# XuyangBai/D3Feat

Hardware: NVIDIA H100
Metric: points/sec through KPFCNN encoder (higher is better)
Workload: dtype f32

## Files before the change

d3feat_b200/csrc/kpconv.cu:

```cuda
#include <stdlib.h>

#include "ops.cuh"

namespace d3f {


constexpr int kS1Warps = 4;
constexpr int kWStride = 20;
constexpr int kKMax = 16;

struct Stage1Params {
  const float* q;
  const float4* s4;
  const int* idx;
  const float* feat;
  int count_nn;
  const float* Kp;
  const float* offsets;
  const float* modulations;
  int Nq, Ns, H, Cin;
  int n0, n1;
  const int* order;
  float extent;
  float inv_scale;
// ... 271 lines not shown
#pragma unroll
        for (int k = 0; k < K; ++k) w[k] = (k == kmin) ? w[k] : 0.f;
      }
      const bool keep = real && qvalid && (!DEFORM || in_range);
#pragma unroll
      for (int kq = 0; kq < KP / 4; ++kq)
        *reinterpret_cast<float4*>(&wq[sl * kWStride + 4 * kq]) =
            keep ? make_float4(w[4 * kq], w[4 * kq + 1], w[4 * kq + 2], w[4 * kq + 3]) : make_float4(0.f, 0.f, 0.f, 0.f);
      if (c0 == 0 && p.count_nn) nn_count += __popc((__ballot_sync(0xffffffffu, sp.w > 0.f) >> gshift) & gmask);
      unsigned m = (__ballot_sync(0xffffffffu, keep) >> gshift) & gmask;
      int cnt = __popc(m);
      if (QPW >= 2) cnt = max(cnt, __shfl_xor_sync(0xffffffffu, cnt, 16));
      if (QPW >= 4) cnt = max(cnt, __shfl_xor_sync(0xffffffffu, cnt, 8));
      __syncwarp();

      constexpr int kUnroll = CPL == 4 ? 2 : 4;
      for (int it = 0; it < cnt; it += kUnroll) {
        int hh[kUnroll];
        float f[kUnroll][CPL];
#pragma unroll
        for (int u = 0; u < kUnroll; ++u) {
          const bool act = m != 0;
          hh[u] = act ? __ffs(m) - 1 : 0;
          m &= m - 1;
          const int idh = __shfl_sync(0xffffffffu, id, (int)gshift + hh[u]);
          const float* fp = p.feat + (size_t)idh * p.Cin + c;
          if (CPL == 4) {
            float4 t = act ? __ldg(reinterpret_cast<const float4*>(fp)) : make_float4(0.f, 0.f, 0.f, 0.f);
            f[u][0] = t.x; f[u][1] = t.y; f[u][2 % CPL] = t.z; f[u][3 % CPL] = t.w;
          } else {
            float2 t = act ? __ldg(reinterpret_cast<const float2*>(fp)) : make_float2(0.f, 0.f);
            f[u][0] = t.x; f[u][1] = t.y;
          }
        }
#pragma unroll
        for (int u = 0; u < kUnroll; ++u) {
          const float4* wp = reinterpret_cast<const float4*>(&wq[hh[u] * kWStride]);
          float2 wpair[KP / 2];
#pragma unroll
          for (int kq = 0; kq < KP / 4; ++kq) {
            float4 t = wp[kq];
            wpair[2 * kq] = make_float2(t.x, t.y);
            wpair[2 * kq + 1] = make_float2(t.z, t.w);
          }
#pragma unroll
          for (int v = 0; v < CPL; ++v) {
            const float2 fd = make_float2(f[u][v], f[u][v]);
#pragma unroll
            for (int j = 0; j < KP / 2; ++j) acc[j][v] = ffma2(wpair[j], fd, acc[j][v]);
          }
        }
      }
      __syncwarp();
    }

    if (qvalid) {
      float* dst = p.wf + (size_t)(n - p.n0) * K * p.Cin + c;
#pragma unroll
      for (int k = 0; k < K; ++k) {
        const float mod = (DEFORM && p.modulations) ? p.modulations[(size_t)nq * K + k] : 1.f;
        float o[CPL];
#pragma unroll
        for (int v = 0; v < CPL; ++v) o[v] = ((k & 1) ? acc[k / 2][v].y : acc[k / 2][v].x) * mod;
        if (CPL == 4) *reinterpret_cast<float4*>(dst + (size_t)k * p.Cin) = make_float4(o[0], o[1], o[2 % CPL], o[3 % CPL]);
        else *reinterpret_cast<float2*>(dst + (size_t)k * p.Cin) = make_float2(o[0], o[1]);
      }
    }
  }
  if (p.inv_nn != nullptr && qvalid && sl == 0) p.inv_nn[n - p.n0] = 1.f / (float)max(nn_count, 1);
}

__device__ __forceinline__ void mma_tf32(float (&c)[4], const unsigned (&a)[4], unsigned b0, unsigned b1) {
  asm volatile("mma.sync.aligned.m16n8k8.row.col.f32.tf32.tf32.f32 {%0,%1,%2,%3}, {%4,%5,%6,%7}, {%8,%9}, {%0,%1,%2,%3};"
               : "+f"(c[0]), "+f"(c[1]), "+f"(c[2]), "+f"(c[3])
               : "r"(a[0]), "r"(a[1]), "r"(a[2]), "r"(a[3]), "r"(b0), "r"(b1));
}
__device__ __forceinline__ void split3(float x, unsigned& hi, unsigned& lo) {
  hi = (__float_as_uint(x) + 0x1000u) & 0xFFFFE000u;
  lo = __float_as_uint(x - __uint_as_float(hi));
}


template <int NT>
__global__ void __launch_bounds__(kS1Warps * 32, NT == 4 ? 8 : (NT == 8 ? 5 : 3))
kpconv_stage1_fast_kernel(Stage1Params p) {
  const int Ns_ = dyn_rows(p.Ns, p.ns_dev), n1_ = min(p.n1, dyn_rows(p.Nq, p.nq_dev));
  constexpr int K = 15;
  static_assert(NT % 4 == 0, "one float4 per four n-tiles");
  const int lane = threadIdx.x & 31, warp = threadIdx.x >> 5;
  const int g = lane >> 2, t = lane & 3;
  const int n = p.n0 + blockIdx.x * kS1Warps + warp;
  if (n >= n1_) return;
  const int kA = g, kB = g + 8;
  const bool validB = kB < K;
  const float kax = p.Kp[3 * kA], kay = p.Kp[3 * kA + 1], kaz = p.Kp[3 * kA + 2];
  const float kbx = validB ? p.Kp[3 * kB] : 1e6f, kby = validB ? p.Kp[3 * kB + 1] : 1e6f,
              kbz = validB ? p.Kp[3 * kB + 2] : 1e6f;
  const int qid = p.order ? p.order[n] : n;
  const float qx = p.q[3 * (size_t)qid], qy = p.q[3 * (size_t)qid + 1], qz = p.q[3 * (size_t)qid + 2];
  const int* row = p.idx + (size_t)qid * p.H + t;
  const float inv_scale = p.inv_scale;
  const unsigned Ns = (unsigned)Ns_;
  const unsigned Cin = (unsigned)p.Cin;
  int cnt = 0;

  constexpr int CCH = NT * 8;
  for (int c0 = blockIdx.y * CCH; c0 < p.Cin; c0 += gridDim.y * CCH) {
    float acc[NT][4];
#pragma unroll
    for (int i = 0; i < NT; ++i) acc[i][0] = acc[i][1] = acc[i][2] = acc[i][3] = 0.f;
    const float* fcol = p.feat + c0 + NT * g;
    asm volatile("" : "+l"(fcol));

    unsigned ida_n = Ns, idb_n = Ns;
    if (t < p.H) ida_n = (unsigned)__ldg(row);
    if (t + 4 < p.H) idb_n = (unsigned)__ldg(row + 4);
    for (int h0 = 0; h0 < p.H; h0 += 8) {
      const unsigned ida = min(ida_n, Ns);
      const unsigned idb = min(idb_n, Ns);
      ida_n = Ns;
      idb_n = Ns;
      if (h0 + 8 + t < p.H) ida_n = (unsigned)__ldg(row + h0 + 8);
      if (h0 + 12 + t < p.H) idb_n = (unsigned)__ldg(row + h0 + 12);
      const float4 spa = __ldg(&p.s4[ida]), spb = __ldg(&p.s4[idb]);
      float fa[NT], fb[NT];
#pragma unroll
      for (int v = 0; v < NT; v += 4) {
        float4 x = make_float4(0.f, 0.f, 0.f, 0.f), y = make_float4(0.f, 0.f, 0.f, 0.f);
        if (ida < Ns) x = __ldg(reinterpret_cast<const float4*>(fcol + (size_t)(ida * Cin) + v));
        if (idb < Ns) y = __ldg(reinterpret_cast<const float4*>(fcol + (size_t)(idb * Cin) + v));
        fa[v] = x.x; fa[v + 1] = x.y; fa[v + 2] = x.z; fa[v + 3] = x.w;
        fb[v] = y.x; fb[v + 1] = y.y; fb[v + 2] = y.z; fb[v + 3] = y.w;
      }
      if (c0 == 0) cnt += (spa.w > 0.f ? 1 : 0) + (spb.w > 0.f ? 1 : 0);
      const float rax = spa.x - qx, ray = spa.y - qy, raz = spa.z - qz;
      const float rbx = spb.x - qx, rby = spb.y - qy, rbz = spb.z - qz;
      auto weight = [&](float rx, float ry, float rz, float kx, float ky, float kz) {
        const float dx = rx - kx, dy = ry - ky, dz = rz - kz;
        const float d2 = fmaf(dz, dz, fmaf(dy, dy, fmaf(dx, dx, 1e-10f)));
        return fmaxf(fmaf(-sqrt_approx(d2), inv_scale, 1.f), 0.f);
      };
      unsigned ah[4], al[4];
      split3(weight(rax, ray, raz, kax, kay, kaz), ah[0], al[0]);
      split3(weight(rax, ray, raz, kbx, kby, kbz), ah[1], al[1]);
      split3(weight(rbx, rby, rbz, kax, kay, kaz), ah[2], al[2]);
      split3(weight(rbx, rby, rbz, kbx, kby, kbz), ah[3], al[3]);
#pragma unroll
      for (int i = 0; i < NT; ++i) {
        unsigned bh0, bl0, bh1, bl1;
        split3(fa[i], bh0, bl0);
        split3(fb[i], bh1, bl1);
        mma_tf32(acc[i], ah, bh0, bh1);
        mma_tf32(acc[i], al, bh0, bh1);
        mma_tf32(acc[i], ah, bl0, bl1);
      }
    }

    float* dst = p.wf + (size_t)(n - p.n0) * K * p.Cin + c0 + 2 * NT * t;
#pragma unroll
    for (int v = 0; v < NT; v += 4) {
      *reinterpret_cast<float4*>(dst + (size_t)kA * p.Cin + v) = make_float4(acc[v][0], acc[v + 1][0], acc[v + 2][0], acc[v + 3][0]);
      *reinterpret_cast<float4*>(dst + (size_t)kA * p.Cin + NT + v) = make_float4(acc[v][1], acc[v + 1][1], acc[v + 2][1], acc[v + 3][1]);
      if (validB) {
        *reinterpret_cast<float4*>(dst + (size_t)kB * p.Cin + v) = make_float4(acc[v][2], acc[v + 1][2], acc[v + 2][2], acc[v + 3][2]);
        *reinterpret_cast<float4*>(dst + (size_t)kB * p.Cin + NT + v) = make_float4(acc[v][3], acc[v + 1][3], acc[v + 2][3], acc[v + 3][3]);
      }
    }
  }
  if (p.inv_nn != nullptr && blockIdx.y == 0) {
    cnt += __shfl_xor_sync(0xffffffffu, cnt, 1);
    cnt += __shfl_xor_sync(0xffffffffu, cnt, 2);
    if (lane == 0) p.inv_nn[n - p.n0] = 1.f / (float)max(cnt, 1);
  }
}

__device__ __forceinline__ uint32_t s1_smem_u32(const void* p) { return (uint32_t)__cvta_generic_to_shared(p); }
__device__ __forceinline__ void s1_cp_async16(uint32_t dst, const void* src, bool valid) {
  const int sz = valid ? 16 : 0;
  asm volatile("cp.async.cg.shared.global [%0], [%1], 16, %2;" ::"r"(dst), "l"(src), "r"(sz) : "memory");
}
__device__ __forceinline__ float4 s1_lds128(uint32_t addr) {
  float4 v;
  asm volatile("ld.shared.v4.f32 {%0, %1, %2, %3}, [%4];" : "=f"(v.x), "=f"(v.y), "=f"(v.z), "=f"(v.w) : "r"(addr));
  return v;
}
template <int NT>
__device__ __forceinline__ int s1_swz(int r3) {
  return NT == 4 ? 2 * r3 : (NT == 8 ? ((r3 & 1) | ((r3 & 2) << 1)) : r3);
}

template <int NT>
__global__ void __launch_bounds__(kS1Warps * 32, NT == 4 ? 8 : (NT == 8 ? 5 : 3))
kpconv_stage1_staged_kernel(Stage1Params p) {
  constexpr int K = 15;
  constexpr int ROWB = NT * 32;
  constexpr int BUFB = 8 * ROWB + 128;
  __shared__ __align__(128) unsigned char stage_sm[kS1Warps][2][BUFB];
  const int Ns_ = dyn_rows(p.Ns, p.ns_dev), n1_ = min(p.n1, dyn_rows(p.Nq, p.nq_dev));
  const int lane = threadIdx.x & 31, warp = threadIdx.x >> 5;
  const int g = lane >> 2, t = lane & 3;
  const int n = p.n0 + blockIdx.x * kS1Warps + warp;
  if (n >= n1_) return;
  const int kA = g, kB = g + 8;
  const bool validB = kB < K;
  const float kax = p.Kp[3 * kA], kay = p.Kp[3 * kA + 1], kaz = p.Kp[3 * kA + 2];
  const float kbx = validB ? p.Kp[3 * kB] : 1e6f, kby = validB ? p.Kp[3 * kB + 1] : 1e6f,
              kbz = validB ? p.Kp[3 * kB + 2] : 1e6f;
  const int qid = p.order ? p.order[n] : n;
  const float qx = p.q[3 * (size_t)qid], qy = p.q[3 * (size_t)qid + 1], qz = p.q[3 * (size_t)qid + 2];
  const int* rowq = p.idx + (size_t)qid * p.H;
  const float inv_scale = p.inv_scale;
  const unsigned Ns = (unsigned)Ns_;
  const unsigned Cin = (unsigned)p.Cin;
  const uint32_t base = s1_smem_u32(&stage_sm[warp][0][0]);
  const int cr = lane >> 3, cc = lane & 7;
  uint32_t wr_row = (uint32_t)(cr * ROWB + (cc ^ s1_swz<NT>(cr & 3)) * 16);
  uint32_t wr_s4 = (uint32_t)(8 * ROWB + lane * 16);
  uint32_t rd_s4 = (uint32_t)(8 * ROWB + t * 16);
  uint32_t rd_row[NT / 4];
#pragma unroll
  for (int v = 0; v < NT; v += 4) {
    const int chunk = g * (NT / 4) + v / 4;
    rd_row[v / 4] = (uint32_t)(t * ROWB + (chunk & ~7) * 16 + (((chunk & 7) ^ s1_swz<NT>(t)) * 16));
    asm volatile("" : "+r"(rd_row[v / 4]));
  }
  asm volatile("" : "+r"(wr_row), "+r"(wr_s4), "+r"(rd_s4));
  int cnt = 0;

  constexpr int CCH = NT * 8;
  for (int c0 = blockIdx.y * CCH; c0 < p.Cin; c0 += gridDim.y * CCH) {
    float acc[NT][4];
#pragma unroll
    for (int i = 0; i < NT; ++i) acc[i][0] = acc[i][1] = acc[i][2] = acc[i][3] = 0.f;
    const float* fsrc = p.feat + c0 + 4 * cc;
    asm volatile("" : "+l"(fsrc));
    auto load_ids = [&](int h0) -> unsigned {
      unsigned v = Ns;
      if (lane < 8 && h0 + lane < p.H) v = (unsigned)__ldg(rowq + h0 + lane);
      return min(v, Ns);
    };
    auto issue = [&](unsigned idv, uint32_t buf) {
      if (lane < 8) s1_cp_async16(buf + wr_s4, p.s4 + idv, true);
      const unsigned i0 = __shfl_sync(0xffffffffu, idv, cr), i1 = __shfl_sync(0xffffffffu, idv, cr + 4);
      const bool ok0 = i0 < Ns, ok1 = i1 < Ns;
      const float* s0 = fsrc + (size_t)((ok0 ? i0 : 0u) * Cin);
      const float* s1 = fsrc + (size_t)((ok1 ? i1 : 0u) * Cin);
#pragma unroll
      for (int seg = 0; seg < ROWB / 128; ++seg) {
        s1_cp_async16(buf + wr_row + seg * 128, s0 + seg * 32, ok0);
        s1_cp_async16(buf + wr_row + 4 * ROWB + seg * 128, s1 + seg * 32, ok1);
      }
    };
    uint32_t cur = base, nxt = base + BUFB;
    unsigned idv_n = load_ids(0);
    issue(idv_n, cur);
    asm volatile("cp.async.commit_group;" ::: "memory");
    idv_n = load_ids(8);
    for (int h0 = 0; h0 < p.H; h0 += 8) {
      if (h0 + 8 < p.H) issue(idv_n, nxt);
      asm volatile("cp.async.commit_group;" ::: "memory");
      idv_n = load_ids(h0 + 16);
      asm volatile("cp.async.wait_group 1;" ::: "memory");
      __syncwarp();
      const float4 spa = s1_lds128(cur + rd_s4), spb = s1_lds128(cur + rd_s4 + 64);
      float fa[NT], fb[NT];
#pragma unroll
      for (int v = 0; v < NT; v += 4) {
        const float4 x = s1_lds128(cur + rd_row[v / 4]), y = s1_lds128(cur + rd_row[v / 4] + 4 * ROWB);
        fa[v] = x.x; fa[v + 1] = x.y; fa[v + 2] = x.z; fa[v + 3] = x.w;
        fb[v] = y.x; fb[v + 1] = y.y; fb[v + 2] = y.z; fb[v + 3] = y.w;
      }
      if (c0 == 0) cnt += (spa.w > 0.f ? 1 : 0) + (spb.w > 0.f ? 1 : 0);
      const float rax = spa.x - qx, ray = spa.y - qy, raz = spa.z - qz;
      const float rbx = spb.x - qx, rby = spb.y - qy, rbz = spb.z - qz;
      auto weight = [&](float rx, float ry, float rz, float kx, float ky, float kz) {
        const float dx = rx - kx, dy = ry - ky, dz = rz - kz;
        const float d2 = fmaf(dz, dz, fmaf(dy, dy, fmaf(dx, dx, 1e-10f)));
        return fmaxf(fmaf(-sqrt_approx(d2), inv_scale, 1.f), 0.f);
      };
      unsigned ah[4], al[4];
      split3(weight(rax, ray, raz, kax, kay, kaz), ah[0], al[0]);
      split3(weight(rax, ray, raz, kbx, kby, kbz), ah[1], al[1]);
      split3(weight(rbx, rby, rbz, kax, kay, kaz), ah[2], al[2]);
      split3(weight(rbx, rby, rbz, kbx, kby, kbz), ah[3], al[3]);
#pragma unroll
      for (int i = 0; i < NT; ++i) {
        unsigned bh0, bl0, bh1, bl1;
        split3(fa[i], bh0, bl0);
        split3(fb[i], bh1, bl1);
        mma_tf32(acc[i], ah, bh0, bh1);
        mma_tf32(acc[i], al, bh0, bh1);
        mma_tf32(acc[i], ah, bl0, bl1);
      }
      __syncwarp();
      const uint32_t tmp = cur;
      cur = nxt;
      nxt = tmp;
    }
    asm volatile("cp.async.wait_group 0;" ::: "memory");

    float* dst = p.wf + (size_t)(n - p.n0) * K * p.Cin + c0 + 2 * NT * t;
#pragma unroll
    for (int v = 0; v < NT; v += 4) {
      *reinterpret_cast<float4*>(dst + (size_t)kA * p.Cin + v) = make_float4(acc[v][0], acc[v + 1][0], acc[v + 2][0], acc[v + 3][0]);
      *reinterpret_cast<float4*>(dst + (size_t)kA * p.Cin + NT + v) = make_float4(acc[v][1], acc[v + 1][1], acc[v + 2][1], acc[v + 3][1]);
      if (validB) {
        *reinterpret_cast<float4*>(dst + (size_t)kB * p.Cin + v) = make_float4(acc[v][2], acc[v + 1][2], acc[v + 2][2], acc[v + 3][2]);
        *reinterpret_cast<float4*>(dst + (size_t)kB * p.Cin + NT + v) = make_float4(acc[v][3], acc[v + 1][3], acc[v + 2][3], acc[v + 3][3]);
      }
    }
  }
  if (p.inv_nn != nullptr && blockIdx.y == 0) {
    cnt += __shfl_xor_sync(0xffffffffu, cnt, 1);
    cnt += __shfl_xor_sync(0xffffffffu, cnt, 2);
    if (lane == 0) p.inv_nn[n - p.n0] = 1.f / (float)max(cnt, 1);
  }
}

template <int NT, bool DEFORM, bool FAST>
__global__ void __launch_bounds__(kS1Warps * 32) kpconv_stage1_mma_kernel(Stage1Params p) {
  const int Ns_ = dyn_rows(p.Ns, p.ns_dev), n1_ = min(p.n1, dyn_rows(p.Nq, p.nq_dev));
  constexpr int K = 15;
  static_assert(NT % 4 == 0, "one float4 per four n-tiles");
  const int lane = threadIdx.x & 31, warp = threadIdx.x >> 5;
  const int g = lane >> 2, t = lane & 3;
  const int n = p.n0 + blockIdx.x * kS1Warps + warp;
  if (n >= n1_) return;
  const int qid = p.order ? p.order[n] : n;
  const int kA = g, kB = g + 8;
  const bool validB = kB < K;
  float kax = p.Kp[3 * kA], kay = p.Kp[3 * kA + 1], kaz = p.Kp[3 * kA + 2];
  float kbx = validB ? p.Kp[3 * kB] : 0.f, kby = validB ? p.Kp[3 * kB + 1] : 0.f, kbz = validB ? p.Kp[3 * kB + 2] : 0.f;
  if (DEFORM) {
    const float* off = p.offsets + (size_t)qid * K * 3;
    kax += off[3 * kA]; kay += off[3 * kA + 1]; kaz += off[3 * kA + 2];
    if (validB) { kbx += off[3 * kB]; kby += off[3 * kB + 1]; kbz += off[3 * kB + 2]; }
  }
  const float qx = p.q[3 * (size_t)qid], qy = p.q[3 * (size_t)qid + 1], qz = p.q[3 * (size_t)qid + 2];
  const int* row = p.idx + (size_t)qid * p.H;
  const float ext2 = p.extent * p.extent;
  const unsigned tmask = 0x11111111u << t;
  int nn_count = 0;

  auto weight = [&](float d2) -> float {
    if (FAST || p.influence == D3F_INFLUENCE_LINEAR) return fmaxf(1.f - sqrt_approx(d2 + 1e-10f) * p.inv_scale, 0.f);
    if (p.influence == D3F_INFLUENCE_GAUSSIAN) return __expf(-d2 * p.gauss_inv);
    return DEFORM ? (d2 < ext2 ? 1.f : 0.f) : 1.f;
  };

  constexpr int CCH = NT * 8;
  for (int c0 = 0; c0 < p.Cin; c0 += CCH) {
    float acc[NT][4];
#pragma unroll
    for (int i = 0; i < NT; ++i) acc[i][0] = acc[i][1] = acc[i][2] = acc[i][3] = 0.f;
    const char* fcol = reinterpret_cast<const char*>(p.feat + c0 + NT * g);
    asm volatile("" : "+l"(fcol));
    const unsigned cin_bytes = (unsigned)p.Cin * 4u;

    for (int h0 = 0; h0 < p.H; h0 += 8) {
      const int ha = h0 + t, hb = h0 + t + 4;
      unsigned ida = ha < p.H ? (unsigned)row[ha] : (unsigned)Ns_, idb = hb < p.H ? (unsigned)row[hb] : (unsigned)Ns_;
      ida = min(ida, (unsigned)Ns_);
      idb = min(idb, (unsigned)Ns_);
      const float4 spa = __ldg(&p.s4[ida]), spb = __ldg(&p.s4[idb]);
      const bool reala = ida < (unsigned)Ns_, realb = idb < (unsigned)Ns_;
      float fa[NT], fb[NT];
#pragma unroll
      for (int v = 0; v < NT; v += 4) {
        float4 x = reala ? __ldg(reinterpret_cast<const float4*>(fcol + (size_t)ida * cin_bytes + 4 * v)) : make_float4(0.f, 0.f, 0.f, 0.f);
        float4 y = realb ? __ldg(reinterpret_cast<const float4*>(fcol + (size_t)idb * cin_bytes + 4 * v)) : make_float4(0.f, 0.f, 0.f, 0.f);
        fa[v] = x.x; fa[v + 1] = x.y; fa[v + 2] = x.z; fa[v + 3] = x.w;
        fb[v] = y.x; fb[v + 1] = y.y; fb[v + 2] = y.z; fb[v + 3] = y.w;
      }
      const float rax = spa.x - qx, ray = spa.y - qy, raz = spa.z - qz;
      const float rbx = spb.x - qx, rby = spb.y - qy, rbz = spb.z - qz;
      float d_aA = (rax - kax) * (rax - kax) + (ray - kay) * (ray - kay) + (raz - kaz) * (raz - kaz);
      float d_aB = (rax - kbx) * (rax - kbx) + (ray - kby) * (ray - kby) + (raz - kbz) * (raz - kbz);
      float d_bA = (rbx - kax) * (rbx - kax) + (rby - kay) * (rby - kay) + (rbz - kaz) * (rbz - kaz);
      float d_bB = (rbx - kbx) * (rbx - kbx) + (rby - kby) * (rby - kby) + (rbz - kbz) * (rbz - kbz);
      float w_aA = weight(d_aA), w_aB = validB ? weight(d_aB) : 0.f;
      float w_bA = weight(d_bA), w_bB = validB ? weight(d_bB) : 0.f;
      if (!FAST && p.closest) {
        float ma = d_aA, mb = d_bA;
        int ia = kA, ib = kA;
        if (validB && d_aB < ma) { ma = d_aB; ia = kB; }
        if (validB && d_bB < mb) { mb = d_bB; ib = kB; }
#pragma unroll
        for (int o = 4; o < 32; o <<= 1) {
          float oa = __shfl_xor_sync(0xffffffffu, ma, o), ob = __shfl_xor_sync(0xffffffffu, mb, o);
          int ja = __shfl_xor_sync(0xffffffffu, ia, o), jb = __shfl_xor_sync(0xffffffffu, ib, o);
          if (oa < ma || (oa == ma && ja < ia)) { ma = oa; ia = ja; }
          if (ob < mb || (ob == mb && jb < ib)) { mb = ob; ib = jb; }
        }
        w_aA = ia == kA ? w_aA : 0.f; w_aB = ia == kB ? w_aB : 0.f;
        w_bA = ib == kA ? w_bA : 0.f; w_bB = ib == kB ? w_bB : 0.f;
      }
      bool keepa = reala, keepb = realb;
      if (DEFORM) {
        const unsigned ra = __ballot_sync(0xffffffffu, d_aA < ext2 || (validB && d_aB < ext2));
        const unsigned rb = __ballot_sync(0xffffffffu, d_bA < ext2 || (validB && d_bB < ext2));
        keepa = keepa && (ra & tmask) != 0;
// ... 225 lines not shown
        wf[k] = fmaf(wk, f, wf[k]);
      }
    }
  } else
  for (int h = sl; h < p.H; h += 8) {
    int id = row[h];
    if (id < 0 || id > Ns_) id = Ns_;
    const float4 sp = __ldg(&p.s4[id]);
    const float f = sp.w, rx = sp.x - qx, ry = sp.y - qy, rz = sp.z - qz;
    nn += f > 0.f ? 1 : 0;
    float w[K];
    float dmin = 3.0e38f;
    int kmin = 0;
#pragma unroll
    for (int k = 0; k < K; ++k) {
      float dx = rx - kp_s[3 * k], dy = ry - kp_s[3 * k + 1], dz = rz - kp_s[3 * k + 2];
      float d2 = dx * dx + dy * dy + dz * dz;
      if (d2 < dmin) { dmin = d2; kmin = k; }
      float wk;
      if (p.influence == D3F_INFLUENCE_LINEAR) wk = fmaxf(1.f - sqrt_approx(d2 + 1e-10f) * p.inv_scale, 0.f);
      else if (p.influence == D3F_INFLUENCE_GAUSSIAN) wk = __expf(-d2 * p.gauss_inv);
      else wk = 1.f;
      w[k] = wk;
    }
#pragma unroll
    for (int k = 0; k < K; ++k) wf[k] += (p.closest && k != kmin) ? 0.f : w[k] * f;
  }
#pragma unroll
  for (int o = 1; o < 8; o <<= 1) {
#pragma unroll
    for (int k = 0; k < K; ++k) wf[k] += __shfl_xor_sync(0xffffffffu, wf[k], o);
    nn += __shfl_xor_sync(0xffffffffu, nn, o);
  }
  if (!qvalid) return;
  const float inv_nn = p.normalize ? 1.f / (float)max(nn, 1) : 1.f;
  for (int c = sl; c < p.Cout; c += 8) {
    float y = 0.f;
#pragma unroll
    for (int k = 0; k < K; ++k) y = fmaf(wf[k], Ws[k * p.Cout + c], y);
    y *= inv_nn;
    if (p.bn_scale) y = fmaf(y, p.bn_scale[c], p.bn_shift[c]);
    if (p.bias) y += p.bias[c];
    if (p.leaky_alpha >= 0.f) y = y > 0.f ? y : y * p.leaky_alpha;
    p.out[(size_t)n * p.Cout + c] = y;
  }
}

struct AuxStream {
  cudaStream_t stream = nullptr;
  cudaEvent_t s1_done[2] = {nullptr, nullptr};
  cudaEvent_t gemm_done[2] = {nullptr, nullptr};
};
constexpr int kMaxDevices = 32;
struct AuxStreams {
  AuxStream dev[kMaxDevices];
  ~AuxStreams() {
    for (int d = 0; d < kMaxDevices; ++d) {
      if (dev[d].stream == nullptr) continue;
      int cur = 0;
      if (cudaGetDevice(&cur) != cudaSuccess || cudaSetDevice(d) != cudaSuccess) continue;
      for (int i = 0; i < 2; ++i) {
        cudaEventDestroy(dev[d].s1_done[i]);
        cudaEventDestroy(dev[d].gemm_done[i]);
      }
      cudaStreamDestroy(dev[d].stream);
      cudaSetDevice(cur);
    }
  }
};
static AuxStream* aux_stream() {
  static thread_local AuxStreams all;
  int dev = 0;
  if (cudaGetDevice(&dev) != cudaSuccess || dev < 0 || dev >= kMaxDevices) return nullptr;
  AuxStream& a = all.dev[dev];
  if (a.stream != nullptr) return &a;
  if (cudaStreamCreateWithFlags(&a.stream, cudaStreamNonBlocking) != cudaSuccess) { a.stream = nullptr; return nullptr; }
  for (int i = 0; i < 2; ++i) {
    cudaEventCreateWithFlags(&a.s1_done[i], cudaEventDisableTiming);
    cudaEventCreateWithFlags(&a.gemm_done[i], cudaEventDisableTiming);
  }
  return &a;
}

static int chunk_queries(int K, int Cin) {
  static const int forced = [] { const char* v = getenv("D3F_KPCONV_CHUNK"); return v ? atoi(v) : 0; }();
  if (forced >= 128) return forced / 128 * 128;
  const long long per = (long long)K * Cin * 4;
  long long n = (512ll << 20) / per;
  if (n < 1024) n = 1024;
  return (int)(n / 128 * 128);
}

size_t kpconv_workspace_bytes(int Nq, int Ns, int H, int K, int Cin, int Cout) {
  (void)H; (void)Cout;
  int chunk = chunk_queries(K, Cin);
  if (chunk > Nq) chunk = Nq > 0 ? Nq : 1;
  size_t b = 0;
  b += 2 * align_up((size_t)chunk * K * Cin * sizeof(float), 256);
  b += 2 * align_up((size_t)chunk * sizeof(float), 256);
  b += align_up((size_t)(Ns + 1) * sizeof(float4), 256);
  b += align_up(tc_gemm_split_ws_floats(chunk, Cout, K * Cin) * sizeof(float), 256);
  b += align_up(kpconv_fused_workspace_bytes(), 256);
  return b + 1024;
}

int kpconv_forward_impl(bool deform, const float* q, const float* s, const int* idx, const float* feat,
                        const float* Kp, const float* offsets, const float* modulations, const float* W,
                        const float* W_packed, const int* query_order, int Nq, int Ns, int H, int K, int Cin, int Cout,
                        float extent,
                        int influence, int mode, int normalize,
                        const float* bn_scale, const float* bn_shift, const float* bias, float leaky_alpha,
                        float* out, void* workspace, size_t workspace_bytes, cudaStream_t stream,
                        const int* nq_dev, const int* ns_dev) {
  D3F_REQUIRE(Nq >= 0 && Ns >= 0 && H >= 0 && Cin >= 1 && Cout >= 1, D3F_ERR_INVALID,
              "kpconv: bad shape Nq=%d Ns=%d H=%d Cin=%d Cout=%d", Nq, Ns, H, Cin, Cout);
  D3F_REQUIRE(K >= 1 && K <= kAnyKMax, D3F_ERR_INVALID, "kpconv: num_kernel_points=%d outside [1, %d]", K, kAnyKMax);
  D3F_REQUIRE(influence >= 0 && influence <= 2, D3F_ERR_INVALID,
              "Unknown influence function type (config.KP_influence)");
  D3F_REQUIRE(mode == D3F_MODE_SUM || mode == D3F_MODE_CLOSEST, D3F_ERR_INVALID,
              "Unknown convolution mode. Should be 'closest' or 'sum'");
  D3F_REQUIRE(extent > 0.f, D3F_ERR_INVALID, "kpconv: KP_extent=%g", (double)extent);
  D3F_REQUIRE((bn_scale == nullptr) == (bn_shift == nullptr), D3F_ERR_INVALID, "kpconv: bn_scale/bn_shift mismatch");
  D3F_REQUIRE(!deform || offsets != nullptr || Nq == 0, D3F_ERR_INVALID, "kpconv_deform: offsets missing");
  D3F_REQUIRE(workspace_bytes >= kpconv_workspace_bytes(Nq, Ns, H, K, Cin, Cout), D3F_ERR_WORKSPACE,
              "kpconv: workspace too small");
  if (Nq == 0) return D3F_OK;
  int chunk = chunk_queries(K, Cin);
  if (chunk > Nq) chunk = Nq;
  Carver cv(workspace, workspace_bytes);
  float* wf_buf[2] = {cv.take<float>((size_t)chunk * K * Cin), cv.take<float>((size_t)chunk * K * Cin)};
  float* nn_buf[2] = {cv.take<float>(chunk), cv.take<float>(chunk)};
  float4* s4 = cv.take<float4>((size_t)Ns + 1);
  size_t split_floats = tc_gemm_split_ws_floats(chunk, Cout, K * Cin);
  float* split_ws = split_floats ? cv.take<float>(split_floats) : nullptr;
  const bool norm = normalize != 0 && !deform;
  {
    const bool first_layer = Cin == 1 && !deform && K == 15;
    int pmode = first_layer ? 2 : (norm ? 1 : 0);
    const float shadow = deform ? 1000.f : 1e6f;
    const bool vec = pmode == 1 && Cin % 4 == 0 && Cin >= 32 && (reinterpret_cast<uintptr_t>(feat) & 15) == 0;
    if (vec && Cin < 64)
      prep_supports_vec_kernel<8><<<ceil_div((Ns + 1) * 8, 256), 256, 0, stream>>>(s, feat, Ns, ns_dev, Cin, shadow, s4);
    else if (vec && Cin < 128)
      prep_supports_vec_kernel<16><<<ceil_div((Ns + 1) * 16, 256), 256, 0, stream>>>(s, feat, Ns, ns_dev, Cin, shadow, s4);
    else if (vec)
      prep_supports_vec_kernel<32><<<ceil_div((Ns + 1) * 32, 256), 256, 0, stream>>>(s, feat, Ns, ns_dev, Cin, shadow, s4);
    else
      prep_supports_kernel<<<ceil_div((Ns + 1) * 32, 256), 256, 0, stream>>>(s, feat, Ns, ns_dev, Cin, pmode, shadow, s4);
    D3F_LAUNCH_CHECK("prep_supports_kernel");
  }
  if (Cin == 1 && !deform && K == 15) {
    Cin1Params c1;
    c1.q = q; c1.s4 = s4; c1.idx = idx; c1.Kp = Kp; c1.W = W;
    c1.Nq = Nq; c1.Ns = Ns; c1.H = H; c1.Cout = Cout;
    c1.inv_scale = 1.f / (2.f * extent);
    float sg = extent * 0.3f;
    c1.gauss_inv = 1.f / (2.f * sg * sg + 1e-9f);
    c1.influence = influence; c1.closest = mode == D3F_MODE_CLOSEST; c1.normalize = normalize != 0;
    c1.shadow = 1e6f;
    c1.bn_scale = bn_scale; c1.bn_shift = bn_shift; c1.bias = bias; c1.leaky_alpha = leaky_alpha;
    c1.order = query_order;
    c1.out = out;
    c1.nq_dev = nq_dev; c1.ns_dev = ns_dev;
    const size_t c1_smem = (size_t)(K * Cout + K * 3) * sizeof(float);
    D3F_REQUIRE(c1_smem <= 48 * 1024, D3F_ERR_CAPACITY, "kpconv (Cin = 1): Cout=%d too wide for the first-layer kernel", Cout);
    if (influence == D3F_INFLUENCE_LINEAR && mode == D3F_MODE_SUM)
      kpconv_cin1_kernel<true><<<ceil_div(ceil_div(Nq, 4) * 32, 256), 256, c1_smem, stream>>>(c1);
    else
      kpconv_cin1_kernel<false><<<ceil_div(ceil_div(Nq, 4) * 32, 256), 256, c1_smem, stream>>>(c1);
    D3F_LAUNCH_CHECK("kpconv_cin1_kernel");
    return D3F_OK;
  }
  if (!deform && W_packed != nullptr &&
      kpconv_fused_supported(Nq, H, K, Cin, Cout, influence, mode, feat, W, out, query_order)) {
    float* w_img = cv.take<float>(kpconv_fused_workspace_bytes() / sizeof(float));
    return kpconv_fused_forward(q, s4, idx, feat, Kp, W, w_img, Nq, Ns, H, Cout, extent, norm ? 1 : 0, bn_scale, bn_shift,
                                bias, leaky_alpha, out, stream, nq_dev, ns_dev);
  }
  Stage1Params p;
  p.q = q; p.s4 = s4; p.idx = idx; p.feat = feat; p.count_nn = norm ? 1 : 0;
  p.Kp = Kp; p.offsets = offsets; p.modulations = modulations;
  p.Nq = Nq; p.Ns = Ns; p.H = H; p.Cin = Cin;
  p.extent = extent;
  p.inv_scale = deform ? 1.f / extent : 1.f / (2.f * extent);
  float sigma = extent * 0.3f;
  p.gauss_inv = 1.f / (2.f * sigma * sigma + 1e-9f);
  p.influence = influence;
  p.closest = mode == D3F_MODE_CLOSEST;
  p.shadow = deform ? 1000.f : 1e6f;
  p.order = query_order;
  p.nq_dev = nq_dev; p.ns_dev = ns_dev;
  const int n_chunks = ceil_div(Nq, chunk);
  AuxStream* aux = n_chunks > 1 ? aux_stream() : nullptr;
  for (int ci = 0, n0 = 0; n0 < Nq; n0 += chunk, ++ci) {
    const int b = ci & 1;
    float* wf = wf_buf[b];
    float* inv_nn = nn_buf[b];
    p.wf = wf;
    p.inv_nn = norm ? inv_nn : nullptr;
    p.n0 = n0;
    p.n1 = min(Nq, n0 + chunk);
    if (aux && ci >= 2) D3F_CUDA(cudaStreamWaitEvent(stream, aux->gemm_done[b], 0));
    int rc = deform ? launch_stage1<true>(K, p, stream) : launch_stage1<false>(K, p, stream);
    if (rc) return rc;
    cudaStream_t gs = stream;
    if (aux) {
      D3F_CUDA(cudaEventRecord(aux->s1_done[b], stream));
      D3F_CUDA(cudaStreamWaitEvent(aux->stream, aux->s1_done[b], 0));
      gs = aux->stream;
    }
    Epilogue ep;
    ep.rowscale = norm ? inv_nn : nullptr;
    ep.bn_scale = bn_scale; ep.bn_shift = bn_shift; ep.bias = bias; ep.residual = nullptr;
    ep.leaky_alpha = leaky_alpha;
    ep.row_map = query_order ? query_order + n0 : nullptr;
    ep.m_dev = nq_dev; ep.m_off = n0;
    float* cbase = query_order ? out : out + (size_t)n0 * Cout;
    if (W_packed != nullptr && tc_gemm_supported(wf, K * Cin))
      rc = tc_gemm(wf, W_packed, cbase, p.n1 - n0, Cout, K * Cin, ep, gs, split_ws);
    else
      rc = gemm_f32(wf, W, cbase, p.n1 - n0, Cout, K * Cin, ep, gs);
    if (rc) return rc;
    if (aux) D3F_CUDA(cudaEventRecord(aux->gemm_done[b], aux->stream));
  }
  if (aux) {
    D3F_CUDA(cudaStreamWaitEvent(stream, aux->gemm_done[0], 0));
    if (n_chunks > 1) D3F_CUDA(cudaStreamWaitEvent(stream, aux->gemm_done[1], 0));
  }
  return D3F_OK;
}

}
```

Measured before the change: 51.98 million.

## Fuse KPConv stage1 and weight contraction for 32-channel layers

Adds a fused kernel for K=15, Cin=Cout=32 linear-sum KPConv layers with many queries. Each block computes the per-kernel-point weighted features for 16 queries into shared memory, then contracts them against a pre-packed hi/lo TF32 weight image with mma. It also applies normalization, batch norm, bias and leaky ReLU and writes the output directly. This removes the global wf workspace round trip, the separate GEMM launch and the chunked two-stream schedule, at the cost of an extra small packing kernel per call and a cross-warp shared-memory reduction.

Measured after the change: 53.59 million (median of 6 runs). 1.03x the previous value.

```diff
diff --git a/d3feat_b200/csrc/kpconv.cu b/d3feat_b200/csrc/kpconv.cu
--- a/d3feat_b200/csrc/kpconv.cu
+++ b/d3feat_b200/csrc/kpconv.cu
@@ -377,6 +377,62 @@
 
 
 template <int NT>
+__device__ __forceinline__ void fast_pass(const Stage1Params& p, const int* row, float qx, float qy, float qz,
+                                          float kax, float kay, float kaz, float kbx, float kby, float kbz,
+                                          unsigned Ns, int c0, int g, int t, float (&acc)[NT][4], int& cnt) {
+  const float inv_scale = p.inv_scale;
+  const unsigned Cin = (unsigned)p.Cin;
+#pragma unroll
+  for (int i = 0; i < NT; ++i) acc[i][0] = acc[i][1] = acc[i][2] = acc[i][3] = 0.f;
+  const float* fcol = p.feat + c0 + NT * g;
+  asm volatile("" : "+l"(fcol));
+
+  unsigned ida_n = Ns, idb_n = Ns;
+  if (t < p.H) ida_n = (unsigned)__ldg(row);
+  if (t + 4 < p.H) idb_n = (unsigned)__ldg(row + 4);
+  for (int h0 = 0; h0 < p.H; h0 += 8) {
+    const unsigned ida = min(ida_n, Ns);
+    const unsigned idb = min(idb_n, Ns);
+    ida_n = Ns;
+    idb_n = Ns;
+    if (h0 + 8 + t < p.H) ida_n = (unsigned)__ldg(row + h0 + 8);
+    if (h0 + 12 + t < p.H) idb_n = (unsigned)__ldg(row + h0 + 12);
+    const float4 spa = __ldg(&p.s4[ida]), spb = __ldg(&p.s4[idb]);
+    float fa[NT], fb[NT];
+#pragma unroll
+    for (int v = 0; v < NT; v += 4) {
+      float4 x = make_float4(0.f, 0.f, 0.f, 0.f), y = make_float4(0.f, 0.f, 0.f, 0.f);
+      if (ida < Ns) x = __ldg(reinterpret_cast<const float4*>(fcol + (size_t)(ida * Cin) + v));
+      if (idb < Ns) y = __ldg(reinterpret_cast<const float4*>(fcol + (size_t)(idb * Cin) + v));
+      fa[v] = x.x; fa[v + 1] = x.y; fa[v + 2] = x.z; fa[v + 3] = x.w;
+      fb[v] = y.x; fb[v + 1] = y.y; fb[v + 2] = y.z; fb[v + 3] = y.w;
+    }
+    if (c0 == 0) cnt += (spa.w > 0.f ? 1 : 0) + (spb.w > 0.f ? 1 : 0);
+    const float rax = spa.x - qx, ray = spa.y - qy, raz = spa.z - qz;
+    const float rbx = spb.x - qx, rby = spb.y - qy, rbz = spb.z - qz;
+    auto weight = [&](float rx, float ry, float rz, float kx, float ky, float kz) {
+      const float dx = rx - kx, dy = ry - ky, dz = rz - kz;
+      const float d2 = fmaf(dz, dz, fmaf(dy, dy, fmaf(dx, dx, 1e-10f)));
+      return fmaxf(fmaf(-sqrt_approx(d2), inv_scale, 1.f), 0.f);
+    };
+    unsigned ah[4], al[4];
+    split3(weight(rax, ray, raz, kax, kay, kaz), ah[0], al[0]);
+    split3(weight(rax, ray, raz, kbx, kby, kbz), ah[1], al[1]);
+    split3(weight(rbx, rby, rbz, kax, kay, kaz), ah[2], al[2]);
+    split3(weight(rbx, rby, rbz, kbx, kby, kbz), ah[3], al[3]);
+#pragma unroll
+    for (int i = 0; i < NT; ++i) {
+      unsigned bh0, bl0, bh1, bl1;
+      split3(fa[i], bh0, bl0);
+      split3(fb[i], bh1, bl1);
+      mma_tf32(acc[i], ah, bh0, bh1);
+      mma_tf32(acc[i], al, bh0, bh1);
+      mma_tf32(acc[i], ah, bl0, bl1);
+    }
+  }
+}
+
+template <int NT>
 __global__ void __launch_bounds__(kS1Warps * 32, NT == 4 ? 8 : (NT == 8 ? 5 : 3))
 kpconv_stage1_fast_kernel(Stage1Params p) {
   const int Ns_ = dyn_rows(p.Ns, p.ns_dev), n1_ = min(p.n1, dyn_rows(p.Nq, p.nq_dev));
@@ -394,62 +450,13 @@
   const int qid = p.order ? p.order[n] : n;
   const float qx = p.q[3 * (size_t)qid], qy = p.q[3 * (size_t)qid + 1], qz = p.q[3 * (size_t)qid + 2];
   const int* row = p.idx + (size_t)qid * p.H + t;
-  const float inv_scale = p.inv_scale;
   const unsigned Ns = (unsigned)Ns_;
-  const unsigned Cin = (unsigned)p.Cin;
   int cnt = 0;
 
   constexpr int CCH = NT * 8;
   for (int c0 = blockIdx.y * CCH; c0 < p.Cin; c0 += gridDim.y * CCH) {
     float acc[NT][4];
-#pragma unroll
-    for (int i = 0; i < NT; ++i) acc[i][0] = acc[i][1] = acc[i][2] = acc[i][3] = 0.f;
-    const float* fcol = p.feat + c0 + NT * g;
-    asm volatile("" : "+l"(fcol));
-
-    unsigned ida_n = Ns, idb_n = Ns;
-    if (t < p.H) ida_n = (unsigned)__ldg(row);
-    if (t + 4 < p.H) idb_n = (unsigned)__ldg(row + 4);
-    for (int h0 = 0; h0 < p.H; h0 += 8) {
-      const unsigned ida = min(ida_n, Ns);
-      const unsigned idb = min(idb_n, Ns);
-      ida_n = Ns;
-      idb_n = Ns;
-      if (h0 + 8 + t < p.H) ida_n = (unsigned)__ldg(row + h0 + 8);
-      if (h0 + 12 + t < p.H) idb_n = (unsigned)__ldg(row + h0 + 12);
-      const float4 spa = __ldg(&p.s4[ida]), spb = __ldg(&p.s4[idb]);
-      float fa[NT], fb[NT];
-#pragma unroll
-      for (int v = 0; v < NT; v += 4) {
-        float4 x = make_float4(0.f, 0.f, 0.f, 0.f), y = make_float4(0.f, 0.f, 0.f, 0.f);
-        if (ida < Ns) x = __ldg(reinterpret_cast<const float4*>(fcol + (size_t)(ida * Cin) + v));
-        if (idb < Ns) y = __ldg(reinterpret_cast<const float4*>(fcol + (size_t)(idb * Cin) + v));
-        fa[v] = x.x; fa[v + 1] = x.y; fa[v + 2] = x.z; fa[v + 3] = x.w;
-        fb[v] = y.x; fb[v + 1] = y.y; fb[v + 2] = y.z; fb[v + 3] = y.w;
-      }
-      if (c0 == 0) cnt += (spa.w > 0.f ? 1 : 0) + (spb.w > 0.f ? 1 : 0);
-      const float rax = spa.x - qx, ray = spa.y - qy, raz = spa.z - qz;
-      const float rbx = spb.x - qx, rby = spb.y - qy, rbz = spb.z - qz;
-      auto weight = [&](float rx, float ry, float rz, float kx, float ky, float kz) {
-        const float dx = rx - kx, dy = ry - ky, dz = rz - kz;
-        const float d2 = fmaf(dz, dz, fmaf(dy, dy, fmaf(dx, dx, 1e-10f)));
-        return fmaxf(fmaf(-sqrt_approx(d2), inv_scale, 1.f), 0.f);
-      };
-      unsigned ah[4], al[4];
-      split3(weight(rax, ray, raz, kax, kay, kaz), ah[0], al[0]);
-      split3(weight(rax, ray, raz, kbx, kby, kbz), ah[1], al[1]);
-      split3(weight(rbx, rby, rbz, kax, kay, kaz), ah[2], al[2]);
-      split3(weight(rbx, rby, rbz, kbx, kby, kbz), ah[3], al[3]);
-#pragma unroll
-      for (int i = 0; i < NT; ++i) {
-        unsigned bh0, bl0, bh1, bl1;
-        split3(fa[i], bh0, bl0);
-        split3(fb[i], bh1, bl1);
-        mma_tf32(acc[i], ah, bh0, bh1);
-        mma_tf32(acc[i], al, bh0, bh1);
-        mma_tf32(acc[i], ah, bl0, bl1);
-      }
-    }
+    fast_pass<NT>(p, row, qx, qy, qz, kax, kay, kaz, kbx, kby, kbz, Ns, c0, g, t, acc, cnt);
 
     float* dst = p.wf + (size_t)(n - p.n0) * K * p.Cin + c0 + 2 * NT * t;
 #pragma unroll
@@ -478,6 +485,9 @@
   float4 v;
   asm volatile("ld.shared.v4.f32 {%0, %1, %2, %3}, [%4];" : "=f"(v.x), "=f"(v.y), "=f"(v.z), "=f"(v.w) : "r"(addr));
   return v;
+}
+__device__ __forceinline__ void s1_sts128(uint32_t addr, float4 v) {
+  asm volatile("st.shared.v4.f32 [%0], {%1, %2, %3, %4};" ::"r"(addr), "f"(v.x), "f"(v.y), "f"(v.z), "f"(v.w) : "memory");
 }
 template <int NT>
 __device__ __forceinline__ int s1_swz(int r3) {
@@ -612,6 +622,152 @@
   }
 }
 
+constexpr int kC32Q = 16;
+constexpr int kC32Stride = 15 * 32 + 16;
+constexpr int kC32RedStride = 40;
+constexpr int kC32ImageFloats = 2 * 15 * 32 * 32;
+constexpr int kC32MinQueries = 16384;
+
+__host__ __device__ __forceinline__ int contract32_image_index(int k, int c) {
+  return (((((k >> 4) * 2) * 4 + (c >> 3)) * 4 + ((c & 7) >> 1)) * 32) + (c & 1) * 16 + (k & 15);
+}
+
+__global__ void __launch_bounds__(256) pack_weight_contract32_kernel(const float* __restrict__ W, float* __restrict__ img) {
+  const int i = blockIdx.x * blockDim.x + threadIdx.x;
+  if (i >= kC32ImageFloats / 2) return;
+  const int k = i >> 5, c = i & 31;
+  unsigned hi, lo;
+  split3(W[i], hi, lo);
+  const int o = contract32_image_index(k, c);
+  img[o] = __uint_as_float(hi);
+  img[o + 16 * 32] = __uint_as_float(lo);
+}
+
+__global__ void __launch_bounds__(kS1Warps * 32, 6)
+kpconv_stage1_contract32_kernel(Stage1Params p, const float* __restrict__ w_img, const float* __restrict__ bn_scale,
+                                const float* __restrict__ bn_shift, const float* __restrict__ bias, float leaky_alpha,
+                                float* __restrict__ out) {
+  constexpr int K = 15;
+  __shared__ __align__(16) float wf_s[kC32Q * kC32Stride];
+  __shared__ float nn_s[kC32Q];
+  static_assert(kS1Warps * kC32Q * kC32RedStride <= kC32Q * kC32Stride, "partial sums reuse the wf tile");
+  const int Ns_ = dyn_rows(p.Ns, p.ns_dev), nq = dyn_rows(p.Nq, p.nq_dev);
+  const int slot0 = blockIdx.x * kC32Q;
+  if (slot0 >= nq) return;
+  const int lane = threadIdx.x & 31, warp = threadIdx.x >> 5;
+  const int g = lane >> 2, t = lane & 3;
+  const uint32_t wf_base = s1_smem_u32(wf_s);
+
+  {
+    const int kA = g, kB = g + 8;
+    const bool validB = kB < K;
+    const float kax = p.Kp[3 * kA], kay = p.Kp[3 * kA + 1], kaz = p.Kp[3 * kA + 2];
+    const float kbx = validB ? p.Kp[3 * kB] : 1e6f, kby = validB ? p.Kp[3 * kB + 1] : 1e6f,
+                kbz = validB ? p.Kp[3 * kB + 2] : 1e6f;
+    for (int i = warp; i < kC32Q; i += kS1Warps) {
+      const int n = slot0 + i;
+      float acc[4][4];
+      int cnt = 0;
+      if (n < nq) {
+        const int qid = p.order ? p.order[n] : n;
+        const float qx = p.q[3 * (size_t)qid], qy = p.q[3 * (size_t)qid + 1], qz = p.q[3 * (size_t)qid + 2];
+        fast_pass<4>(p, p.idx + (size_t)qid * p.H + t, qx, qy, qz, kax, kay, kaz, kbx, kby, kbz, (unsigned)Ns_, 0, g, t,
+                     acc, cnt);
+      } else {
+#pragma unroll
+        for (int v = 0; v < 4; ++v) acc[v][0] = acc[v][1] = acc[v][2] = acc[v][3] = 0.f;
+      }
+      const uint32_t rowa = wf_base + (uint32_t)(i * kC32Stride + 32 * kA) * 4u;
+      const uint32_t rowb = wf_base + (uint32_t)(i * kC32Stride + 32 * kB) * 4u;
+      const uint32_t sw = (uint32_t)(kA & 1);
+      s1_sts128(rowa + ((2 * t) ^ sw) * 16u, make_float4(acc[0][0], acc[1][0], acc[2][0], acc[3][0]));
+      s1_sts128(rowa + ((2 * t + 1) ^ sw) * 16u, make_float4(acc[0][1], acc[1][1], acc[2][1], acc[3][1]));
+      if (validB) {
+        s1_sts128(rowb + ((2 * t) ^ sw) * 16u, make_float4(acc[0][2], acc[1][2], acc[2][2], acc[3][2]));
+        s1_sts128(rowb + ((2 * t + 1) ^ sw) * 16u, make_float4(acc[0][3], acc[1][3], acc[2][3], acc[3][3]));
+      }
+      cnt += __shfl_xor_sync(0xffffffffu, cnt, 1);
+      cnt += __shfl_xor_sync(0xffffffffu, cnt, 2);
+      if (lane == 0) nn_s[i] = p.count_nn ? 1.f / (float)max(cnt, 1) : 1.f;
+    }
+  }
+  __syncthreads();
+
+  float sum[4][4];
+#pragma unroll
+  for (int nt = 0; nt < 4; ++nt) sum[nt][0] = sum[nt][1] = sum[nt][2] = sum[nt][3] = 0.f;
+  const uint32_t arow0 = wf_base + (uint32_t)(g * kC32Stride) * 4u, arow1 = arow0 + 8u * kC32Stride * 4u;
+  const float* wl = w_img + contract32_image_index(4 * t, g);
+  for (int kp = warp; kp < K; kp += kS1Warps) {
+    float part[4][4];
+#pragma unroll
+    for (int nt = 0; nt < 4; ++nt) part[nt][0] = part[nt][1] = part[nt][2] = part[nt][3] = 0.f;
+#pragma unroll
+    for (int b = 0; b < 2; ++b) {
+      const uint32_t col = (uint32_t)(32 * kp + 4 * ((4 * b + t) ^ (kp & 1))) * 4u;
+      const float4 x0 = s1_lds128(arow0 + col), x1 = s1_lds128(arow1 + col);
+      unsigned ah[2][4], al[2][4];
+      split3(x0.x, ah[0][0], al[0][0]);
+      split3(x1.x, ah[0][1], al[0][1]);
+      split3(x0.y, ah[0][2], al[0][2]);
+      split3(x1.y, ah[0][3], al[0][3]);
+      split3(x0.z, ah[1][0], al[1][0]);
+      split3(x1.z, ah[1][1], al[1][1]);
+      split3(x0.w, ah[1][2], al[1][2]);
+      split3(x1.w, ah[1][3], al[1][3]);
+#pragma unroll
+      for (int nt = 0; nt < 4; ++nt) {
+        const float* bp = wl + (2 * kp + b) * 1024 + nt * 128;
+        const float4 bh = __ldg(reinterpret_cast<const float4*>(bp));
+        const float4 bl = __ldg(reinterpret_cast<const float4*>(bp + 16 * 32));
+        mma_tf32(part[nt], ah[0], __float_as_uint(bh.x), __float_as_uint(bh.y));
+        mma_tf32(part[nt], al[0], __float_as_uint(bh.x), __float_as_uint(bh.y));
+        mma_tf32(part[nt], ah[0], __float_as_uint(bl.x), __float_as_uint(bl.y));
+        mma_tf32(part[nt], ah[1], __float_as_uint(bh.z), __float_as_uint(bh.w));
+        mma_tf32(part[nt], al[1], __float_as_uint(bh.z), __float_as_uint(bh.w));
+        mma_tf32(part[nt], ah[1], __float_as_uint(bl.z), __float_as_uint(bl.w));
+      }
+    }
+#pragma unroll
+    for (int nt = 0; nt < 4; ++nt)
+#pragma unroll
+      for (int e = 0; e < 4; ++e) sum[nt][e] += part[nt][e];
+  }
+  __syncthreads();
+
+  float* red = wf_s;
+#pragma unroll
+  for (int nt = 0; nt < 4; ++nt) {
+    *reinterpret_cast<float2*>(&red[(warp * kC32Q + g) * kC32RedStride + 8 * nt + 2 * t]) = make_float2(sum[nt][0], sum[nt][1]);
+    *reinterpret_cast<float2*>(&red[(warp * kC32Q + g + 8) * kC32RedStride + 8 * nt + 2 * t]) = make_float2(sum[nt][2], sum[nt][3]);
+  }
+  __syncthreads();
+
+  const int r = threadIdx.x >> 3, c = (threadIdx.x & 7) * 4;
+  const int n = slot0 + r;
+  if (n >= nq) return;
+  float y[4];
+  {
+    const float4 s = *reinterpret_cast<const float4*>(&red[r * kC32RedStride + c]);
+    y[0] = s.x; y[1] = s.y; y[2] = s.z; y[3] = s.w;
+  }
+#pragma unroll
+  for (int w = 1; w < kS1Warps; ++w) {
+    const float4 s = *reinterpret_cast<const float4*>(&red[(w * kC32Q + r) * kC32RedStride + c]);
+    y[0] += s.x; y[1] += s.y; y[2] += s.z; y[3] += s.w;
+  }
+  const float rs = nn_s[r];
+#pragma unroll
+  for (int e = 0; e < 4; ++e) {
+    y[e] *= rs;
+    if (bn_scale) y[e] = fmaf(y[e], bn_scale[c + e], bn_shift[c + e]);
+    if (bias) y[e] += bias[c + e];
+    if (leaky_alpha >= 0.f) y[e] = y[e] > 0.f ? y[e] : y[e] * leaky_alpha;
+  }
+  const size_t orow = p.order ? (size_t)p.order[n] : (size_t)n;
+  *reinterpret_cast<float4*>(out + orow * 32 + c) = make_float4(y[0], y[1], y[2], y[3]);
+}
+
 template <int NT, bool DEFORM, bool FAST>
 __global__ void __launch_bounds__(kS1Warps * 32) kpconv_stage1_mma_kernel(Stage1Params p) {
   const int Ns_ = dyn_rows(p.Ns, p.ns_dev), n1_ = min(p.n1, dyn_rows(p.Nq, p.nq_dev));
@@ -1003,13 +1159,29 @@
   return &a;
 }
 
+static int forced_chunk() {
+  static const int forced = [] { const char* v = getenv("D3F_KPCONV_CHUNK"); return v ? atoi(v) : 0; }();
+  return forced >= 128 ? forced / 128 * 128 : 0;
+}
 static int chunk_queries(int K, int Cin) {
-  static const int forced = [] { const char* v = getenv("D3F_KPCONV_CHUNK"); return v ? atoi(v) : 0; }();
-  if (forced >= 128) return forced / 128 * 128;
+  if (forced_chunk()) return forced_chunk();
   const long long per = (long long)K * Cin * 4;
   long long n = (512ll << 20) / per;
   if (n < 1024) n = 1024;
   return (int)(n / 128 * 128);
+}
+
+static bool contract32_path(bool deform, int Nq, int Ns, int K, int Cin, int Cout, int influence, int mode,
+                            const float* feat, const float* W_packed, const float* out) {
+  if (deform || K != 15 || Cin != 32 || Cout != 32 || influence != D3F_INFLUENCE_LINEAR || mode != D3F_MODE_SUM ||
+      Nq < kC32MinQueries || W_packed == nullptr || (long long)(Ns + 1) * Cin >= (1ll << 31))
+    return false;
+  if (((reinterpret_cast<uintptr_t>(feat) | reinterpret_cast<uintptr_t>(out)) & 15) != 0) return false;
+  const char* fused = getenv("D3F_FUSED_KPCONV");
+  const char* staged = getenv("D3F_S1_STAGED");
+  const char* pared = getenv("D3F_S1_PARED");
+  return !(fused && fused[0] == '0') && !(staged && atoi(staged) != 0) && !(pared && pared[0] == '0') &&
+         forced_chunk() == 0;
 }
 
 size_t kpconv_workspace_bytes(int Nq, int Ns, int H, int K, int Cin, int Cout) {
@@ -1111,6 +1283,19 @@
   p.shadow = deform ? 1000.f : 1e6f;
   p.order = query_order;
   p.nq_dev = nq_dev; p.ns_dev = ns_dev;
+  if (contract32_path(deform, Nq, Ns, K, Cin, Cout, influence, mode, feat, W_packed, out)) {
+    p.wf = nullptr; p.inv_nn = nullptr;
+    p.n0 = 0; p.n1 = Nq;
+    D3F_REQUIRE(kpconv_fused_workspace_bytes() >= kC32ImageFloats * sizeof(float), D3F_ERR_WORKSPACE,
+                "kpconv: the weight image buffer is too small");
+    float* w_img = cv.take<float>(kpconv_fused_workspace_bytes() / sizeof(float));
+    pack_weight_contract32_kernel<<<ceil_div(kC32ImageFloats / 2, 256), 256, 0, stream>>>(W, w_img);
+    D3F_LAUNCH_CHECK("pack_weight_contract32_kernel");
+    kpconv_stage1_contract32_kernel<<<ceil_div(Nq, kC32Q), kS1Warps * 32, 0, stream>>>(p, w_img, bn_scale, bn_shift,
+                                                                                        bias, leaky_alpha, out);
+    D3F_LAUNCH_CHECK("kpconv_stage1_contract32_kernel");
+    return D3F_OK;
+  }
   const int n_chunks = ceil_div(Nq, chunk);
   AuxStream* aux = n_chunks > 1 ? aux_stream() : nullptr;
   for (int ci = 0, n0 = 0; n0 < Nq; n0 += chunk, ++ci) {
```
